# Leqr/MSMP-PDE

Measured on AMD Instinct MI355X. Metric: rollout-steps/sec (whole node), E2 nx=100 tw=25, higher is better.
Workload: dtype f32; 1 GPU; E2 MSMP-PDE (MP_PDE_SolverLEMLinGated), 2048 graphs x nx=100, time_window=25, 6 gated layer pairs, radius graph n=3; graphs_total=2048, graphs_per_gpu=2048, nodes_per_gpu=204800, edges_per_gpu=1204224, parallelism=dp1 (graph-sharded, no collective in the rollout), sub_batches=1, range_policy_switched_to_exact_fp32=False, preheat=163 untimed steps (>= 1 s) after the 5 warm-up steps

## Files before the change

### msmp-pde_amd/csrc/aux_kernels.hip

```cpp
#include <limits.h>
#include <stdarg.h>
#include <string.h>
#include "graph_norm.h"
#include <vector>
#include "mfma_tiles.h"

namespace msmp {

static thread_local char g_err[512] = "";

void set_error(const char* fmt, ...) {
    va_list ap;
    va_start(ap, fmt);
    vsnprintf(g_err, sizeof(g_err), fmt, ap);
    va_end(ap);
}

int check_launch(const char* what) {
    const hipError_t e = hipGetLastError();
    if (e != hipSuccess) {
        set_error("%s: %s", what, hipGetErrorString(e));
        return MSMP_ERR_HIP;
    }
    return MSMP_OK;
// ... 354 lines not shown
            (void)hipGetLastError();
            if (hipMalloc(&dp, sizeof(int)) == hipSuccess && hipMemset(dp, 0, sizeof(int)) == hipSuccess) {
                g_status_dev = static_cast<int*>(dp);
                g_status_mode = 2;
            } else {
                (void)hipGetLastError();
                g_status_mode = -1;
            }
        }
    }
    return g_status_dev;
}
}

extern "C" int msmp_last_status(int* flags_out, int reset) {
    MSMP_REQUIRE(flags_out, MSMP_ERR_ARG, "msmp_last_status: null pointer");
    int* dp = status_ptr();
    *flags_out = 0;
    if (g_status_mode == 1) {
        *flags_out = __atomic_load_n(g_status_host, __ATOMIC_RELAXED);
        if (reset) __atomic_store_n(g_status_host, 0, __ATOMIC_RELAXED);
    } else if (g_status_mode == 2) {
        hipError_t e = hipMemcpy(flags_out, dp, sizeof(int), hipMemcpyDeviceToHost);
        if (e == hipSuccess && reset) e = hipMemset(dp, 0, sizeof(int));
        MSMP_REQUIRE(e == hipSuccess, MSMP_ERR_HIP, "msmp_last_status: %s", hipGetErrorString(e));
    } else {
        MSMP_REQUIRE(false, MSMP_ERR_HIP, "msmp_last_status: no status word (allocation failed)");
    }
    return MSMP_OK;
}

extern "C" int msmp_version(void) { return MSMP_ABI_VERSION; }
extern "C" const char* msmp_last_error(void) { return g_err; }

struct TuneRow {
    const char* key;
    int value;
    int def;
    int lo, hi;
    bool flag;
    constexpr TuneRow(const char* k, int d, int l, int h, bool f) : key(k), value(d), def(d), lo(l), hi(h), flag(f) {}
};
#define ANY_INT INT_MIN, INT_MAX, false
#define ON_OFF INT_MIN, INT_MAX, true
static TuneRow g_tune[] = {
    {"split", 1, ANY_INT},
    {"edge_nb", 0, ANY_INT},
    {"pair", 1, ANY_INT},
    {"tile", 2, ANY_INT},
    {"tile_arith", 1, ANY_INT},
    {"tile_align", 0, ANY_INT},
    {"bwd_gemm", 1, ANY_INT},
    {"tail", 1, ANY_INT},
    {"lem_share", 1, 1, 16, false},
    {"lem_tail", 1, ON_OFF},
    {"lem_wide", 1, ON_OFF},
    {"wide_msg", 1, ON_OFF},
    {"wide_tail", 0, ON_OFF},
    {"wide_proj", 0, ON_OFF},
};
#undef ANY_INT
#undef ON_OFF

static TuneRow* tune_row(const char* key) {
    if (key)
        for (TuneRow& r : g_tune)
            if (!strcmp(key, r.key)) return &r;
    return nullptr;
}

int msmp_tune_get(const char* key) {
    const TuneRow* r = tune_row(key);
    return r ? r->value : 0;
}

extern "C" int msmp_tune_query(const char* key) { return msmp_tune_get(key); }

extern "C" int msmp_tune(const char* key, int value) {
    TuneRow* r = tune_row(key);
    MSMP_REQUIRE(r, MSMP_ERR_ARG, "msmp_tune: unknown key");
    MSMP_REQUIRE(value >= r->lo && value <= r->hi, MSMP_ERR_ARG, "msmp_tune: %s = %d is out of range (%d to %d)", key, value, r->lo, r->hi);
    r->value = r->flag ? value != 0 : value;
    return MSMP_OK;
}

extern "C" int64_t msmp_packed_layer_floats(int tw, int nv) {
    if (tw <= 0 || nv < 1 || nv > MSMP_MAX_VARS) return -1;
    return packed_layout(tw, nv).total;
}

extern "C" int msmp_pack_layer_f32(const float* w1, const float* b1, const float* w2, const float* b2,
                                   const float* w3, const float* b3, const float* w4, const float* b4,
                                   int tw, int nv, float* packed_out, msmp_stream_t stream) {
    MSMP_REQUIRE(w1 && b1 && w2 && b2 && w3 && b3 && w4 && b4 && packed_out, MSMP_ERR_ARG, "msmp_pack_layer_f32: null pointer");
    MSMP_REQUIRE(tw > 0 && nv >= 1 && nv <= MSMP_MAX_VARS, MSMP_ERR_ARG, "msmp_pack_layer_f32: bad tw=%d nv=%d", tw, nv);
    PackArgs a{w1, b1, w2, b2, w3, b3, w4, b4, tw, nv, packed_out};
    hipLaunchKernelGGL(pack_layer_kernel, dim3(256), dim3(256), 0, (hipStream_t)stream, a);
    hipLaunchKernelGGL(pack_layer_scale_kernel, dim3(4), dim3(256), 0, (hipStream_t)stream, a);
    hipLaunchKernelGGL(pack_layer_split_kernel, dim3(256), dim3(256), 0, (hipStream_t)stream, a);
    return check_launch("pack_layer_kernel");
}

extern "C" int msmp_scatter_mean_f32(const float* msg, const int32_t* rowptr, int64_t n_nodes, float* agg_out,
                                     msmp_stream_t stream) {
    MSMP_REQUIRE(rowptr && agg_out, MSMP_ERR_ARG, "msmp_scatter_mean_f32: null pointer");
    MSMP_REQUIRE(n_nodes > 0 && n_nodes < (1L << 31), MSMP_ERR_ARG, "msmp_scatter_mean_f32: bad n_nodes");
// ... 130 lines not shown
```

### msmp-pde_amd/csrc/mlp_kernels.hip

```cpp
#include "mfma_tiles.h"

namespace msmp {

struct EdgeArgs {
    const float* h;
    const float* u;
    const float* pos;
    const float* vars;
    const int* tgt;
    const int* col;
    const int* rowptr;
    long n_edges, n_nodes;
    int tile_nodes;
    int xcd_map;
    int tw, nv, nc1;
    const float* w1;
    const float* w2;
    const float* w2s;
    const float* scales;
    const float* b1;
    const float* b2;
    const float* P;
    const float* Q;
    float* msg;
// ... 783 lines not shown
        }
    }
#pragma unroll
    for (int T = 0; T < 4; ++T)
#pragma unroll
        for (int r = 0; r < 16; ++r) y[T][0][r] *= inv4;
}

__global__ __launch_bounds__(256, 2) void node_update_split_kernel(NodeSplitArgs sa) {
    __shared__ __attribute__((aligned(16))) float lds[2 * SPLIT_CHUNK_FLOATS];
    const NodeArgs& a = sa.b;
    const int tid = threadIdx.x, lane = tid & 63, wave = tid >> 6;
    const int c = lane & 31, hh = lane >> 5;
    const long n = (long)blockIdx.x * 128 + wave * 32 + c;
    const long nc = n < a.n_nodes ? n : a.n_nodes - 1;
    f32x16 y[4][1];
    node_head_split(a.h, a.agg, a.vars, nc, a.nv, a.b3, a.b4, a.w3v, sa.w3s, sa.scales, lds, tid, lane, hh, y);
    if (n < a.n_nodes) {
        float* o = a.out + (size_t)n * H + 4 * hh;
        const float* hx = a.h + (size_t)n * H + 4 * hh;
#pragma unroll
        for (int T = 0; T < 4; ++T)
#pragma unroll
            for (int q = 0; q < 4; ++q) {
                f32x4 v;
                if (a.mode == MSMP_LAYER_LIN) {
#pragma unroll
                    for (int m = 0; m < 4; ++m) v[m] = y[T][0][4 * q + m];
                } else {
                    const f32x4 x = *reinterpret_cast<const f32x4*>(hx + 32 * T + 8 * q);
#pragma unroll
                    for (int m = 0; m < 4; ++m) v[m] = x[m] + swishf(y[T][0][4 * q + m]);
                }
                *reinterpret_cast<f32x4*>(o + 32 * T + 8 * q) = v;
            }
    }
}

struct TailArgs {
    const float* h;
    const float* agg[2];
    const float* vars;
    const int* graph_ptr;
    int nv, mode;
    float eps;
    const float* b3[2];
    const float* b4[2];
    const float* w3vh[2];
    const float* w3s[2];
    const float* w4t[2];
    const float* scales[2];
    float* out;
    int* status;
};

constexpr float TAIL_ACT_SCALE = 64.0f;
constexpr float TAIL_NODE_SCALE = 256.0f;
__device__ __forceinline__ float tail_node_scaled(float x) { return __builtin_amdgcn_fmed3f(x * TAIL_NODE_SCALE, -65504.0f, 65504.0f); }

constexpr int ROWBUF_FLOATS = 128 * 32;
__device__ __forceinline__ void tail_rows_issue(const float* __restrict__ h, const float* __restrict__ agg, int n0, int n1, int ch, float* buf, int tid) {
    const float* src = (ch < 4 ? h : agg) + 32 * (ch & 3);
#pragma unroll
    for (int i = 0; i < 4; ++i) {
        const int P = tid + 256 * i, r = P >> 3;
        const int node = min(n0 + r, n1 - 1);
        const float* g = src + (size_t)node * H + 4 * ((P & 7) ^ ((r >> 1) & 7));
        __builtin_amdgcn_global_load_lds((const __attribute__((address_space(1))) void*)g, (__attribute__((address_space(3))) void*)(buf + 4 * P), 16, 0, 0);
    }
}
__device__ __forceinline__ void tail_rows_read(const float* buf, int row, int hh, f32x4 (&dst)[4]) {
    const float* rb = buf + row * 32;
    const int sw = (row >> 1) & 7;
#pragma unroll
    for (int s = 0; s < 2; ++s) {
        dst[2 * s] = *reinterpret_cast<const f32x4*>(rb + 4 * ((4 * s + 2 * hh) ^ sw));
        dst[2 * s + 1] = *reinterpret_cast<const f32x4*>(rb + 4 * ((4 * s + 2 * hh + 1) ^ sw));
    }
}

__device__ __forceinline__ void wstage_dma(const float* __restrict__ chunk, float* buf, int tid) {
#pragma unroll
    for (int i = 0; i < 4; ++i)
        __builtin_amdgcn_global_load_lds((const __attribute__((address_space(1))) void*)(chunk + 4 * (tid + 256 * i)),
                                         (__attribute__((address_space(3))) void*)(buf + 4 * (tid + 256 * i)), 16, 0, 0);
}

__device__ __forceinline__ void tail_bias_load(const float* b3, int hh, f32x16 (&z)[4][1]) {
#pragma unroll
    for (int T = 0; T < 4; ++T)
#pragma unroll
        for (int q = 0; q < 4; ++q) {
            const f32x4 bv = *reinterpret_cast<const f32x4*>(b3 + 32 * T + 8 * q + 4 * hh);
#pragma unroll
            for (int m = 0; m < 4; ++m) z[T][0][4 * q + m] = bv[m];
        }
}
__device__ __forceinline__ void tail_bias_pin(f32x16 (&z)[4][1]) {
#pragma unroll
    for (int T = 0; T < 4; ++T) asm volatile("" : "+v"(z[T][0]));
}
__device__ __forceinline__ void tail_bias_scale(f32x16 (&z)[4][1], float sc3) {
#pragma unroll
    for (int T = 0; T < 4; ++T)
#pragma unroll
        for (int r = 0; r < 16; ++r) z[T][0][r] *= sc3;
}
__device__ __forceinline__ float tail_sc3(const float* scales) { return uniform_ro(scales, 2) * TAIL_NODE_SCALE; }

__device__ __forceinline__ void tail_chunk_frags(const float* buf, int myrow, int hh, half8 (&bhi)[1][2], half8 (&blo)[1][2]) {
    f32x4 pf[4];
    tail_rows_read(buf, myrow, hh, pf);
#pragma unroll
    for (int s = 0; s < 2; ++s) {
        const f32x4 v0 = pf[2 * s], v1 = pf[2 * s + 1];
        const float v[8] = {v0[0], v0[1], v0[2], v0[3], v1[0], v1[1], v1[2], v1[3]};
        split8_node(v, bhi[0][s], blo[0][s]);
    }
}

template <int CH0, int PB>
__device__ __forceinline__ void head_chunks(float* rowbuf, int n0, int n1, const float* __restrict__ h, const float* __restrict__ agg, const float* w3vh,
                                            const float* w3s, const float* w4t, float* lds, int tid, int lane, int myrow, int hh, f32x16 (&z)[4][1],
                                            half8 (&wvf)[2][4] PROF_ARGS) {
#pragma unroll
    for (int ch = CH0; ch < 8; ++ch) {
        if (ch < 7) tail_rows_issue(h, agg, n0, n1, ch + 1, rowbuf + ((ch + 1) & 1) * ROWBUF_FLOATS, tid);
        wstage_dma(ch < 7 ? w3s + (size_t)(ch + 1) * SPLIT_CHUNK_FLOATS : w4t, lds + ((ch + 1) & 1) * SPLIT_CHUNK_FLOATS, tid);
        half8 bhi[1][2], blo[1][2];
        tail_chunk_frags(rowbuf + (ch & 1) * ROWBUF_FLOATS, myrow, hh, bhi, blo);
        if (ch == 5) {
            const half8* wv = reinterpret_cast<const half8*>(w3vh) + lane;
#pragma unroll
            for (int m = 0; m < 2; ++m)
#pragma unroll
                for (int T = 0; T < 4; ++T) wvf[m][T] = wv[(m * 4 + T) * 64];
        }
        PROF_MARK(PB);
        mma_chunk_split<1>(lds + (ch & 1) * SPLIT_CHUNK_FLOATS, lane, bhi, blo, z);
        PROF_MARK(PB + 1);
        __syncthreads();
        PROF_MARK(PB + 2);
    }
}

__device__ __forceinline__ void tail_var_frags(const float* xvl, int myrow, int hh, half8 (&bx)[2]) {
    const f32x4 x0 = *reinterpret_cast<const f32x4*>(xvl + 8 * myrow), x1 = *reinterpret_cast<const f32x4*>(xvl + 8 * myrow + 4);
    const float xr[8] = {x0[0], x0[1], x0[2], x0[3], x1[0], x1[1], x1[2], x1[3]};
    float xv[8];
#pragma unroll
    for (int f = 0; f < 8; ++f) xv[f] = tail_node_scaled(xr[f]);
    var_slot_frags(xv, hh, bx);
}

template <typename MidHook, typename LastHook>
__device__ __forceinline__ void head_finish(const float* b4, const float* w4t, const float* scales, float* lds, int tid, int lane, int c, int hh,
                                            f32x16 (&z)[4][1], const half8 (&wvf)[2][4], const half8 (&bx)[2], f32x16 (&yT)[4], MidHook mid_hook,
                                            LastHook last_hook, bool center, float* zref) {
    const float inv3 = uniform_ro(scales, 6) * (TAIL_ACT_SCALE / TAIL_NODE_SCALE), sc4 = uniform_ro(scales, 3) * TAIL_ACT_SCALE;
#pragma unroll
    for (int m = 0; m < 2; ++m)
#pragma unroll
        for (int T = 0; T < 4; ++T) z[T][0] = __builtin_amdgcn_mfma_f32_32x32x16_f16(wvf[m][T], bx[m], z[T][0], 0, 0, 0);
    mid_hook();
    __builtin_amdgcn_sched_barrier(0);
#pragma unroll
    for (int T = 0; T < 4; ++T)
#pragma unroll
        for (int r = 0; r < 16; ++r) {
#if MSMP_PRECISE_ACT
            z[T][0][r] = TAIL_ACT_SCALE * swishf(z[T][0][r] * inv3 * (1.0f / TAIL_ACT_SCALE));
#else
            const float xs = z[T][0][r] * inv3;
            const float e = __builtin_amdgcn_exp2f(xs * (-1.44269504088896340736f / TAIL_ACT_SCALE));
            z[T][0][r] = xs * __builtin_amdgcn_rcpf(1.0f + e);
#endif
        }

    if (center) {
        if ((tid >> 6) == 0 && c == 0) {
#pragma unroll
            for (int T = 0; T < 4; ++T)
#pragma unroll
                for (int q = 0; q < 4; ++q)
                    *reinterpret_cast<f32x4*>(zref + 32 * T + 8 * q + 4 * hh) = f32x4{z[T][0][4 * q], z[T][0][4 * q + 1], z[T][0][4 * q + 2], z[T][0][4 * q + 3]};
        }
        __syncthreads();
#pragma unroll
        for (int T = 0; T < 4; ++T)
#pragma unroll
            for (int q = 0; q < 4; ++q) {
                const f32x4 rv = *reinterpret_cast<const f32x4*>(zref + 32 * T + 8 * q + 4 * hh);
#pragma unroll
                for (int m = 0; m < 4; ++m) z[T][0][4 * q + m] -= rv[m];
            }
    }
    {
        const f32x4 bv = center ? f32x4{0.f, 0.f, 0.f, 0.f} : *reinterpret_cast<const f32x4*>(b4 + 4 * c) * sc4;
#pragma unroll
        for (int T = 0; T < 4; ++T)
#pragma unroll
            for (int r = 0; r < 16; ++r) yT[T][r] = bv[T];
    }
#pragma unroll
    for (int t = 0; t < 4; ++t) {
        if (t < 3) wstage_dma(w4t + (size_t)(t + 1) * SPLIT_CHUNK_FLOATS, lds + ((t + 1) & 1) * SPLIT_CHUNK_FLOATS, tid);
        else last_hook();
        __builtin_amdgcn_sched_barrier(0);
        half8 zhi[1][2], zlo[1][2];
        split_acc_tile<1>(z[t], zhi, zlo);
        const half8* w = reinterpret_cast<const half8*>(lds + (t & 1) * SPLIT_CHUNK_FLOATS) + lane;
#pragma unroll
        for (int s = 0; s < 2; ++s)
#pragma unroll
            for (int T = 0; T < 4; ++T) {
                const half8 whi = w[((s * 4 + T) * 2 + 0) * 64], wlo = w[((s * 4 + T) * 2 + 1) * 64];
                MSMP_MFMA_LOLO(1, yT[T], zlo[0][s], wlo);
                yT[T] = __builtin_amdgcn_mfma_f32_32x32x16_f16(zhi[0][s], wlo, yT[T], 0, 0, 0);
                yT[T] = __builtin_amdgcn_mfma_f32_32x32x16_f16(zlo[0][s], whi, yT[T], 0, 0, 0);
                yT[T] = __builtin_amdgcn_mfma_f32_32x32x16_f16(zhi[0][s], whi, yT[T], 0, 0, 0);
            }
        if (t < 3) __syncthreads();
    }
}

__device__ __forceinline__ void tile_t_total(const float (&v)[4], float* part, float* tot, int tid, int wave, int c, int hh,
                                             float (&out)[4]) {
#pragma unroll
    for (int T = 0; T < 4; ++T) part[(wave * 2 + hh) * H + 32 * T + c] = v[T];
    __syncthreads();
    if (tid < H) {
        float s = 0.f;
#pragma unroll
        for (int p = 0; p < 8; ++p) s += part[p * H + tid];
        tot[tid] = s;
    }
    __syncthreads();
#pragma unroll
    for (int T = 0; T < 4; ++T) out[T] = tot[32 * T + c];
}

__device__ __forceinline__ void tile_t_instance_norm(f32x16 (&x)[4], int wave, int cnt, float unit, float eps, float* part, float* tot,
                                                     int tid, int c, int hh, int* status) {
    const float inv = 1.0f / (float)max(cnt, 1);
    const bool ragged = wave * 32 + 32 > cnt;
    if (ragged) {
#pragma unroll
        for (int T = 0; T < 4; ++T)
#pragma unroll
            for (int r = 0; r < 16; ++r) x[T][r] = wave * 32 + acc_row(r, hh) < cnt ? x[T][r] : 0.f;
    }
    float s[4], m[4];
#pragma unroll
    for (int T = 0; T < 4; ++T) {
        float a0 = 0.f, a1 = 0.f;
#pragma unroll
        for (int r = 0; r < 16; r += 2) { a0 += x[T][r]; a1 += x[T][r + 1]; }
        s[T] = a0 + a1;
    }
    tile_t_total(s, part, tot, tid, wave, c, hh, m);
#pragma unroll
    for (int T = 0; T < 4; ++T) {
        const float mean = m[T] * inv;
        float a0 = 0.f, a1 = 0.f;
#pragma unroll
        for (int r = 0; r < 16; r += 2) {
            x[T][r] -= mean;
            x[T][r + 1] -= mean;
            if (ragged) {
                x[T][r] = wave * 32 + acc_row(r, hh) < cnt ? x[T][r] : 0.f;
                x[T][r + 1] = wave * 32 + acc_row(r + 1, hh) < cnt ? x[T][r + 1] : 0.f;
            }
            a0 = fmaf(x[T][r], x[T][r], a0);
            a1 = fmaf(x[T][r + 1], x[T][r + 1], a1);
        }
        s[T] = a0 + a1;
    }
    tile_t_total(s, part, tot, tid, wave, c, hh, m);
    if (wave == 0 && !(m[0] + m[1] + m[2] + m[3] < 3.0e38f)) status_raise(status, MSMP_STATUS_NONFINITE);
#pragma unroll
    for (int T = 0; T < 4; ++T) {
        const float f = unit * msmp_rsq(m[T] * inv * unit * unit + eps);
#pragma unroll
        for (int r = 0; r < 16; ++r) x[T][r] *= f;
    }
}

template <bool GATED>
__global__ __launch_bounds__(256, 2) void node_tail_split_kernel(TailArgs a) {
    __shared__ __attribute__((aligned(16))) float smem[2 * SPLIT_CHUNK_FLOATS + 2 * ROWBUF_FLOATS + 9 * H + 8 * 128];
    float* const lds = smem;
    float* const rowbuf = smem + 2 * SPLIT_CHUNK_FLOATS;
    float* const part = rowbuf + 2 * ROWBUF_FLOATS;
    float* const tot = part + 8 * H;
    float* const xvl = tot + H;
    const int tid = threadIdx.x, lane = tid & 63, wave = tid >> 6;
    const int c = lane & 31, hh = lane >> 5;
    const int n0 = a.graph_ptr[blockIdx.x], n1 = a.graph_ptr[blockIdx.x + 1];
    const int cnt = n1 - n0;
    if (cnt <= 0) return;

    PROF_DECL
#pragma unroll
    for (int i = 0; i < 4; ++i) {
        const int e = tid + 256 * i, row = e >> 3, f = e & 7;
        const float v = a.vars[(size_t)min(n0 + row, n1 - 1) * a.nv + min(f, a.nv - 1)];
        xvl[e] = v * (row < cnt && f < a.nv ? 1.0f : 0.f);
    }
    const int myrow = wave * 32 + c;
    f32x16 tau[4], y[4];
    f32x16 z[4][1];
    half8 wvf[2][4], bx[2];
    if (GATED) {
        f32x16 zg[4][1];
        tail_rows_issue(a.h, a.agg[1], n0, n1, 0, rowbuf, tid);
        wstage_dma(a.w3s[1], lds, tid);
        tail_bias_load(a.b3[1], hh, zg);
        tail_bias_load(a.b3[0], hh, z);
        tail_bias_pin(zg);
        tail_bias_pin(z);
        tail_bias_scale(zg, tail_sc3(a.scales[1]));
        tail_bias_scale(z, tail_sc3(a.scales[0]));
        __syncthreads();
        PROF_MARK(5);
        half8 bhi[1][2], blo[1][2];
#pragma unroll
        for (int s = 0; s < 8; ++s) {
            const int ch = s >> 1;
            if (!(s & 1)) {
                tail_rows_issue(a.h, a.agg[1], n0, n1, ch + 1, rowbuf + ((ch + 1) & 1) * ROWBUF_FLOATS, tid);
                wstage_dma(a.w3s[0] + (size_t)ch * SPLIT_CHUNK_FLOATS, lds + SPLIT_CHUNK_FLOATS, tid);
                __builtin_amdgcn_sched_barrier(0);
                tail_chunk_frags(rowbuf + (ch & 1) * ROWBUF_FLOATS, myrow, hh, bhi, blo);
                PROF_MARK(6);
                mma_chunk_split<1>(lds, lane, bhi, blo, zg);
            } else {
                wstage_dma(a.w3s[1] + (size_t)(ch + 1) * SPLIT_CHUNK_FLOATS, lds, tid);
                __builtin_amdgcn_sched_barrier(0);
                PROF_MARK(6);
                mma_chunk_split<1>(lds + SPLIT_CHUNK_FLOATS, lane, bhi, blo, z);
            }
            PROF_MARK(7);
            __syncthreads();
            PROF_MARK(8);
        }
        head_chunks<4, 9>(rowbuf, n0, n1, a.h, a.agg[1], a.w3vh[1], a.w3s[1], a.w4t[1], lds, tid, lane, myrow, hh, zg, wvf PROF_PASS);
        tail_var_frags(xvl, myrow, hh, bx);
        head_finish(a.b4[1], a.w4t[1], a.scales[1], lds, tid, lane, c, hh, zg, wvf, bx, tau,
                    [&] { tail_rows_issue(a.h, a.agg[0], n0, n1, 4, rowbuf, tid); },
                    [&] { wstage_dma(a.w3s[0] + (size_t)4 * SPLIT_CHUNK_FLOATS, lds, tid); }, true, tot);
        PROF_MARK(0);
        tile_t_instance_norm(tau, wave, cnt, uniform_ro(a.scales[1], 7) * (1.0f / TAIL_ACT_SCALE), a.eps, part, tot, tid, c, hh, a.status);
#pragma unroll
        for (int T = 0; T < 4; ++T)
#pragma unroll
            for (int r = 0; r < 16; ++r) tau[T][r] = sigmoidf_(tau[T][r]);
        __syncthreads();
        PROF_MARK(1);
        head_chunks<4, 12>(rowbuf, n0, n1, a.h, a.agg[0], a.w3vh[0], a.w3s[0], a.w4t[0], lds, tid, lane, myrow, hh, z, wvf PROF_PASS);
    } else {
        tail_rows_issue(a.h, a.agg[0], n0, n1, 0, rowbuf, tid);
        wstage_dma(a.w3s[0], lds, tid);
        tail_bias_load(a.b3[0], hh, z);
        tail_bias_pin(z);
        tail_bias_scale(z, tail_sc3(a.scales[0]));
        __syncthreads();
        PROF_MARK(5);
        head_chunks<0, 12>(rowbuf, n0, n1, a.h, a.agg[0], a.w3vh[0], a.w3s[0], a.w4t[0], lds, tid, lane, myrow, hh, z, wvf PROF_PASS);
        tail_var_frags(xvl, myrow, hh, bx);
    }
    head_finish(a.b4[0], a.w4t[0], a.scales[0], lds, tid, lane, c, hh, z, wvf, bx, y, [] {}, [] {}, GATED || a.mode == MSMP_LAYER_LIN, tot);
    PROF_MARK(2);
    const size_t base = ((size_t)n0 + wave * 32 + 4 * hh) * H + 4 * c;
    const int lim = cnt - wave * 32 - 4 * hh;
    const bool full = wave * 32 + 32 <= cnt;
    const bool need_h = GATED || a.mode != MSMP_LAYER_LIN;
    f32x4 hx[16];
    if (need_h) {
        if (full) {
#pragma unroll
            for (int r = 0; r < 16; ++r) hx[r] = *reinterpret_cast<const f32x4*>(a.h + base + (size_t)((r & 3) + 8 * (r >> 2)) * H);
        } else {
#pragma unroll
            for (int r = 0; r < 16; ++r) {
                const int row = (r & 3) + 8 * (r >> 2);
                hx[r] = row < lim ? *reinterpret_cast<const f32x4*>(a.h + base + (size_t)row * H) : f32x4{0.f, 0.f, 0.f, 0.f};
            }
        }
    }
    float unit = uniform_ro(a.scales[0], 7) * (1.0f / TAIL_ACT_SCALE);
    if (!GATED && a.mode != MSMP_LAYER_LIN) {
#pragma unroll
        for (int T = 0; T < 4; ++T)
#pragma unroll
            for (int r = 0; r < 16; ++r) y[T][r] = hx[r][T] + swishf(y[T][r] * unit);
        unit = 1.0f;
    }
    tile_t_instance_norm(y, wave, cnt, unit, a.eps, part, tot, tid, c, hh, a.status);
    if (need_h) {
        float mx = 0.f;
#pragma unroll
        for (int r = 0; r < 16; ++r) mx = fmaxf(fmaxf(fmaxf(fabsf(hx[r][0]), fabsf(hx[r][1])), fmaxf(fabsf(hx[r][2]), fabsf(hx[r][3]))), mx);
        if (mx > NODE_RANGE) status_raise(a.status, MSMP_STATUS_NODE_SATURATED);
    }
    PROF_MARK(3);
    if (GATED) {
#pragma unroll
        for (int T = 0; T < 4; ++T)
#pragma unroll
            for (int r = 0; r < 16; ++r) y[T][r] = fmaf(tau[T][r], swishf(y[T][r]) - hx[r][T], hx[r][T]);
    }
    if (full) {
#pragma unroll
        for (int r = 0; r < 16; ++r)
            *reinterpret_cast<f32x4*>(a.out + base + (size_t)((r & 3) + 8 * (r >> 2)) * H) = f32x4{y[0][r], y[1][r], y[2][r], y[3][r]};
    } else {
#pragma unroll
        for (int r = 0; r < 16; ++r) {
            const int row = (r & 3) + 8 * (r >> 2);
            if (row < lim) *reinterpret_cast<f32x4*>(a.out + base + (size_t)row * H) = f32x4{y[0][r], y[1][r], y[2][r], y[3][r]};
        }
    }
    PROF_MARK(4);
    PROF_FLUSH
}

}

using namespace msmp;


extern "C" int msmp_edge_mlp_f32(const float* h, const float* u, const float* pos, const float* vars,
                                 const int32_t* tgt, const int32_t* col, int64_t n_nodes, int64_t n_edges,
                                 int tw, int nv, const float* packed, float* msg_out, msmp_stream_t stream) {
    MSMP_REQUIRE(h && u && pos && vars && tgt && col && packed && msg_out, MSMP_ERR_ARG, "msmp_edge_mlp_f32: null pointer");
    MSMP_REQUIRE(n_nodes > 0 && n_edges >= 0 && tw > 0 && nv >= 1 && nv <= MSMP_MAX_VARS, MSMP_ERR_ARG,
                 "msmp_edge_mlp_f32: bad sizes N=%ld E=%ld tw=%d nv=%d", (long)n_nodes, (long)n_edges, tw, nv);
    MSMP_REQUIRE(n_edges < (1L << 31) && n_nodes < (1L << 31), MSMP_ERR_UNSUPPORTED, "msmp_edge_mlp_f32: int32 index range");
    if (n_edges == 0) return MSMP_OK;
    const PackedLayout L = packed_layout(tw, nv);
    EdgeArgs a{h, u, pos, vars, tgt, col, nullptr, (long)n_edges, (long)n_nodes, 0, 0, tw, nv, L.nc1,
               packed + L.w1, packed + L.w2, packed + L.w2s, packed + L.scales, packed + L.b1, packed + L.b2, nullptr, nullptr, msg_out, nullptr, msmp_tune_get("split") ? status_ptr() : nullptr};
    constexpr int NB = 2;
    const unsigned grid = (unsigned)((n_edges + 128 * NB - 1) / (128 * NB));
    timing_begin(MSMP_K_EDGE_MLP, (hipStream_t)stream);
    hipLaunchKernelGGL((edge_mlp_kernel<NB, false, false>), dim3(grid), dim3(256), 0, (hipStream_t)stream, a);
    timing_end(MSMP_K_EDGE_MLP, (hipStream_t)stream);
    return check_launch("edge_mlp_kernel");
}

extern "C" int msmp_node_project_f32(const float* h, const float* u, const float* pos, const float* vars, int64_t n_nodes,
                                     int tw, int nv, const float* packed, float* p_out, float* q_out, msmp_stream_t stream) {
    MSMP_REQUIRE(h && u && pos && vars && packed && p_out && q_out, MSMP_ERR_ARG, "msmp_node_project_f32: null pointer");
    MSMP_REQUIRE(n_nodes > 0 && n_nodes < (1L << 31) && tw > 0 && nv >= 1 && nv <= MSMP_MAX_VARS, MSMP_ERR_ARG,
                 "msmp_node_project_f32: bad sizes");
    const PackedLayout L = packed_layout(tw, nv);
    ProjArgs a{h, u, pos, vars, (long)n_nodes, tw, nv, L.nc1, packed + L.w1, packed + L.b1, p_out, q_out};
    const unsigned grid = (unsigned)((n_nodes + 127) / 128);
    timing_begin(MSMP_K_NODE_PROJ, (hipStream_t)stream);
    if (msmp_tune_get("split")) {
        ProjSplitArgs sa{a, packed + L.w1t, packed + L.scales};
        hipLaunchKernelGGL(node_proj_split_kernel, dim3(grid), dim3(256), 0, (hipStream_t)stream, sa);
    } else
        hipLaunchKernelGGL(node_proj_kernel, dim3(grid), dim3(256), 0, (hipStream_t)stream, a);
    timing_end(MSMP_K_NODE_PROJ, (hipStream_t)stream);
    return check_launch("node_proj_kernel");
}

constexpr int64_t PAIR_MAX_NODES = 65536;

static int edge_aggregate(const float* h, const float* u, const float* pos, const float* vars, const float* P, const float* Q,
                          const int32_t* rowptr, const int32_t* col, const int32_t* tgt, int64_t n_nodes, int64_t n_edges,
                          int max_in_degree, int tw, int nv, const float* packed, float* agg_out, msmp_stream_t stream,
                          const char* who) {
    MSMP_REQUIRE(rowptr && col && tgt && packed && agg_out, MSMP_ERR_ARG, "%s: null pointer", who);
    MSMP_REQUIRE(n_nodes > 0 && n_edges >= 0 && tw > 0 && nv >= 1 && nv <= MSMP_MAX_VARS && max_in_degree >= 0, MSMP_ERR_ARG,
                 "%s: bad sizes", who);
// ... 30 lines not shown
    if (!pair || (pair == 1 && n_nodes > PAIR_MAX_NODES)) return MSMP_ERR_UNSUPPORTED;
    if (!msmp_tune_get("split") || msmp_tune_get("edge_nb") == 2) return MSMP_ERR_UNSUPPORTED;
    if (n_edges <= 0 || max_in_degree <= 0 || max_in_degree > 128 || n_edges >= (1L << 31) || n_nodes >= (1L << 31)) return MSMP_ERR_UNSUPPORTED;
    const PackedLayout L = packed_layout(tw, nv);
    hipStream_t st = (hipStream_t)stream;
    ProjSplitArgs2 pa;
    const float* packed[2] = {packed_a, packed_b};
    float* pp[2] = {p_a, p_b};
    float* qq[2] = {q_a, q_b};
    float* agg[2] = {agg_a, agg_b};
    for (int i = 0; i < 2; ++i)
        pa.head[i] = ProjSplitArgs{ProjArgs{h, u, pos, vars, (long)n_nodes, tw, nv, L.nc1, packed[i] + L.w1, packed[i] + L.b1, pp[i], qq[i]},
                                   packed[i] + L.w1t, packed[i] + L.scales};
    timing_begin(MSMP_K_NODE_PROJ, st);
    hipLaunchKernelGGL(node_proj_split_pair_kernel, dim3((unsigned)((n_nodes + 127) / 128), 2), dim3(256), 0, st, pa);
    timing_end(MSMP_K_NODE_PROJ, st);
    int tile_nodes = 128 / max_in_degree;
    if (tile_nodes > 256) tile_nodes = 256;
    EdgeArgs2 ea;
    for (int i = 0; i < 2; ++i)
        ea.head[i] = EdgeArgs{nullptr, nullptr, nullptr, nullptr, tgt, col, rowptr, (long)n_edges, (long)n_nodes, tile_nodes, 0, tw, nv, L.nc1,
                              packed[i] + L.w1, packed[i] + L.w2, packed[i] + L.w2s, packed[i] + L.scales, packed[i] + L.b1,
                              packed[i] + L.b2, pp[i], qq[i], nullptr, agg[i], status_ptr()};
    timing_begin(MSMP_K_EDGE_MLP, st);
    hipLaunchKernelGGL(edge_mlp_pair_kernel_occ2, dim3((unsigned)((n_nodes + tile_nodes - 1) / tile_nodes), 2), dim3(256), 0, st, ea);
    timing_end(MSMP_K_EDGE_MLP, st);
    return check_launch("edge_mlp_pair_kernel_occ2");
}

extern "C" int msmp_edge_aggregate_f32(const float* h, const float* u, const float* pos, const float* vars,
                                       const int32_t* rowptr, const int32_t* col, const int32_t* tgt, int64_t n_nodes,
                                       int64_t n_edges, int max_in_degree, int tw, int nv, const float* packed,
                                       float* agg_out, msmp_stream_t stream) {
    MSMP_REQUIRE(h && u && pos && vars, MSMP_ERR_ARG, "msmp_edge_aggregate_f32: null pointer");
    return edge_aggregate(h, u, pos, vars, nullptr, nullptr, rowptr, col, tgt, n_nodes, n_edges, max_in_degree, tw, nv, packed,
                          agg_out, stream, "msmp_edge_aggregate_f32");
}

extern "C" int msmp_edge_aggregate_projected_f32(const float* p, const float* q, const int32_t* rowptr, const int32_t* col,
                                                 const int32_t* tgt, int64_t n_nodes, int64_t n_edges, int max_in_degree,
                                                 int tw, int nv, const float* packed, float* agg_out, msmp_stream_t stream) {
    MSMP_REQUIRE(p && q, MSMP_ERR_ARG, "msmp_edge_aggregate_projected_f32: null pointer");
    return edge_aggregate(nullptr, nullptr, nullptr, nullptr, p, q, rowptr, col, tgt, n_nodes, n_edges, max_in_degree, tw, nv,
                          packed, agg_out, stream, "msmp_edge_aggregate_projected_f32");
}

#if MSMP_PROF
extern "C" __attribute__((visibility("default"))) int msmp_debug_prof(unsigned long long* out16, int reset) {
    if (reset) { unsigned long long z[16] = {0}; return (int)hipMemcpyToSymbol(HIP_SYMBOL(g_prof), z, sizeof(z)); }
    return (int)hipMemcpyFromSymbol(out16, HIP_SYMBOL(g_prof), 16 * sizeof(unsigned long long));
}
#endif

extern "C" int msmp_node_tail_f32(const float* h, const float* agg_main, const float* agg_gate, const float* vars,
                                  const int32_t* graph_ptr, int64_t n_nodes, int64_t n_graphs, int max_graph_nodes, int nv,
                                  const float* packed_main, const float* packed_gate, int mode, float eps, float* out,
                                  msmp_stream_t stream) {
    MSMP_REQUIRE(h && agg_main && vars && graph_ptr && packed_main && out, MSMP_ERR_ARG, "msmp_node_tail_f32: null pointer");
    MSMP_REQUIRE((agg_gate != nullptr) == (packed_gate != nullptr), MSMP_ERR_ARG, "msmp_node_tail_f32: give both gate arguments or none");
    MSMP_REQUIRE(n_nodes > 0 && n_graphs > 0 && n_graphs < (1L << 31) && nv >= 1 && nv <= MSMP_MAX_VARS, MSMP_ERR_ARG,
                 "msmp_node_tail_f32: bad sizes");
    MSMP_REQUIRE(mode == MSMP_LAYER_LIN || mode == MSMP_LAYER_RESIDUAL_SWISH, MSMP_ERR_ARG, "msmp_node_tail_f32: bad mode %d", mode);
    MSMP_REQUIRE(!packed_gate || mode == MSMP_LAYER_LIN, MSMP_ERR_ARG, "msmp_node_tail_f32: the gated pair uses GNN_LayerLin layers");
    MSMP_REQUIRE(out != h, MSMP_ERR_ARG, "msmp_node_tail_f32: out may not alias h");
    MSMP_REQUIRE(max_graph_nodes > 0 && max_graph_nodes <= 128, MSMP_ERR_UNSUPPORTED,
                 "msmp_node_tail_f32: graphs of up to 128 nodes (got max_graph_nodes=%d); use the piecewise entry points", max_graph_nodes);
    MSMP_REQUIRE(msmp_tune_get("split"), MSMP_ERR_UNSUPPORTED, "msmp_node_tail_f32: only on the fp16-split matrix path");
    const PackedLayout L = packed_layout(1, nv);
    const float* pg = packed_gate ? packed_gate : packed_main;
    TailArgs a{h, {agg_main, agg_gate}, vars, graph_ptr, nv, mode, eps,
               {packed_main + L.b3, pg + L.b3}, {packed_main + L.b4, pg + L.b4}, {packed_main + L.w3vh, pg + L.w3vh},
               {packed_main + L.w3s, pg + L.w3s}, {packed_main + L.w4t, pg + L.w4t}, {packed_main + L.scales, pg + L.scales}, out, status_ptr()};
    timing_begin(MSMP_K_NODE_UPDATE, (hipStream_t)stream);
    if (packed_gate) hipLaunchKernelGGL(node_tail_split_kernel<true>, dim3((unsigned)n_graphs), dim3(256), 0, (hipStream_t)stream, a);
    else hipLaunchKernelGGL(node_tail_split_kernel<false>, dim3((unsigned)n_graphs), dim3(256), 0, (hipStream_t)stream, a);
    timing_end(MSMP_K_NODE_UPDATE, (hipStream_t)stream);
    return check_launch("node_tail_split_kernel");
}

extern "C" int msmp_node_update_f32(const float* h, const float* agg, const float* vars, int64_t n_nodes, int nv,
                                    const float* packed, int mode, float* out, msmp_stream_t stream) {
    MSMP_REQUIRE(h && agg && vars && packed && out, MSMP_ERR_ARG, "msmp_node_update_f32: null pointer");
    MSMP_REQUIRE(n_nodes > 0 && nv >= 1 && nv <= MSMP_MAX_VARS, MSMP_ERR_ARG, "msmp_node_update_f32: bad sizes");
    MSMP_REQUIRE(mode == MSMP_LAYER_LIN || mode == MSMP_LAYER_RESIDUAL_SWISH, MSMP_ERR_ARG, "msmp_node_update_f32: bad mode %d", mode);
    MSMP_REQUIRE(out != h, MSMP_ERR_ARG, "msmp_node_update_f32: out may not alias h");
    const PackedLayout L = packed_layout(1, nv);
    NodeArgs a{h, agg, vars, (long)n_nodes, nv, mode, packed + L.w3, packed + L.w4,
               packed + L.b3, packed + L.b4, packed + L.w3v, out};
    constexpr int NB = 1;
    const unsigned grid = (unsigned)((n_nodes + 128 * NB - 1) / (128 * NB));
    timing_begin(MSMP_K_NODE_UPDATE, (hipStream_t)stream);
    if (msmp_tune_get("split")) {
        NodeSplitArgs sa{a, packed + L.w3s, packed + L.scales};
        hipLaunchKernelGGL(node_update_split_kernel, dim3(grid), dim3(256), 0, (hipStream_t)stream, sa);
    } else
        hipLaunchKernelGGL(node_update_kernel<NB>, dim3(grid), dim3(256), 0, (hipStream_t)stream, a);
    timing_end(MSMP_K_NODE_UPDATE, (hipStream_t)stream);
    return check_launch("node_update_kernel");
}
```

Baseline: 161.4 rollout-steps/s.

## Make node tail kernel persistent with next-graph prologue prefetch

```diff
diff --git a/msmp-pde_amd/csrc/aux_kernels.hip b/msmp-pde_amd/csrc/aux_kernels.hip
--- a/msmp-pde_amd/csrc/aux_kernels.hip
+++ b/msmp-pde_amd/csrc/aux_kernels.hip
@@ -430,6 +430,7 @@
     {"tile_align", 0, ANY_INT},
     {"bwd_gemm", 1, ANY_INT},
     {"tail", 1, ANY_INT},
+    {"tail_grid", 0, 0, INT_MAX, false},
     {"lem_share", 1, 1, 16, false},
     {"lem_tail", 1, ON_OFF},
     {"lem_wide", 1, ON_OFF},
diff --git a/msmp-pde_amd/csrc/mlp_kernels.hip b/msmp-pde_amd/csrc/mlp_kernels.hip
--- a/msmp-pde_amd/csrc/mlp_kernels.hip
+++ b/msmp-pde_amd/csrc/mlp_kernels.hip
@@ -859,6 +859,7 @@
     const float* scales[2];
     float* out;
     int* status;
+    unsigned n_graphs;
 };
 
 constexpr float TAIL_ACT_SCALE = 64.0f;
@@ -867,12 +868,12 @@
 
 constexpr int ROWBUF_FLOATS = 128 * 32;
 __device__ __forceinline__ void tail_rows_issue(const float* __restrict__ h, const float* __restrict__ agg, int n0, int n1, int ch, float* buf, int tid) {
-    const float* src = (ch < 4 ? h : agg) + 32 * (ch & 3);
+    const float* src = (ch < 4 ? h : agg) + (size_t)n0 * H + 32 * (ch & 3);
 #pragma unroll
     for (int i = 0; i < 4; ++i) {
         const int P = tid + 256 * i, r = P >> 3;
-        const int node = min(n0 + r, n1 - 1);
-        const float* g = src + (size_t)node * H + 4 * ((P & 7) ^ ((r >> 1) & 7));
+        const unsigned row = (unsigned)min(r, n1 - n0 - 1);
+        const float* g = src + (row * (unsigned)H + 4u * (unsigned)((P & 7) ^ ((r >> 1) & 7)));
         __builtin_amdgcn_global_load_lds((const __attribute__((address_space(1))) void*)g, (__attribute__((address_space(3))) void*)(buf + 4 * P), 16, 0, 0);
     }
 }
@@ -893,26 +894,6 @@
                                          (__attribute__((address_space(3))) void*)(buf + 4 * (tid + 256 * i)), 16, 0, 0);
 }
 
-__device__ __forceinline__ void tail_bias_load(const float* b3, int hh, f32x16 (&z)[4][1]) {
-#pragma unroll
-    for (int T = 0; T < 4; ++T)
-#pragma unroll
-        for (int q = 0; q < 4; ++q) {
-            const f32x4 bv = *reinterpret_cast<const f32x4*>(b3 + 32 * T + 8 * q + 4 * hh);
-#pragma unroll
-            for (int m = 0; m < 4; ++m) z[T][0][4 * q + m] = bv[m];
-        }
-}
-__device__ __forceinline__ void tail_bias_pin(f32x16 (&z)[4][1]) {
-#pragma unroll
-    for (int T = 0; T < 4; ++T) asm volatile("" : "+v"(z[T][0]));
-}
-__device__ __forceinline__ void tail_bias_scale(f32x16 (&z)[4][1], float sc3) {
-#pragma unroll
-    for (int T = 0; T < 4; ++T)
-#pragma unroll
-        for (int r = 0; r < 16; ++r) z[T][0][r] *= sc3;
-}
 __device__ __forceinline__ float tail_sc3(const float* scales) { return uniform_ro(scales, 2) * TAIL_NODE_SCALE; }
 
 __device__ __forceinline__ void tail_chunk_frags(const float* buf, int myrow, int hh, half8 (&bhi)[1][2], half8 (&blo)[1][2]) {
@@ -934,6 +915,7 @@
     for (int ch = CH0; ch < 8; ++ch) {
         if (ch < 7) tail_rows_issue(h, agg, n0, n1, ch + 1, rowbuf + ((ch + 1) & 1) * ROWBUF_FLOATS, tid);
         wstage_dma(ch < 7 ? w3s + (size_t)(ch + 1) * SPLIT_CHUNK_FLOATS : w4t, lds + ((ch + 1) & 1) * SPLIT_CHUNK_FLOATS, tid);
+        __builtin_amdgcn_sched_barrier(0);
         half8 bhi[1][2], blo[1][2];
         tail_chunk_frags(rowbuf + (ch & 1) * ROWBUF_FLOATS, myrow, hh, bhi, blo);
         if (ch == 5) {
@@ -951,12 +933,12 @@
     }
 }
 
-__device__ __forceinline__ void tail_var_frags(const float* xvl, int myrow, int hh, half8 (&bx)[2]) {
+__device__ __forceinline__ void tail_var_frags(const float* xvl, int myrow, int hh, int cnt, int nv, half8 (&bx)[2]) {
     const f32x4 x0 = *reinterpret_cast<const f32x4*>(xvl + 8 * myrow), x1 = *reinterpret_cast<const f32x4*>(xvl + 8 * myrow + 4);
     const float xr[8] = {x0[0], x0[1], x0[2], x0[3], x1[0], x1[1], x1[2], x1[3]};
     float xv[8];
 #pragma unroll
-    for (int f = 0; f < 8; ++f) xv[f] = tail_node_scaled(xr[f]);
+    for (int f = 0; f < 8; ++f) xv[f] = tail_node_scaled(xr[f] * (myrow < cnt && f < nv ? 1.0f : 0.f));
     var_slot_frags(xv, hh, bx);
 }
 
@@ -1031,18 +1013,19 @@
     }
 }
 
+__device__ __forceinline__ void tail_lds_barrier() { asm volatile("s_waitcnt lgkmcnt(0)\n\ts_barrier" ::: "memory"); }
 __device__ __forceinline__ void tile_t_total(const float (&v)[4], float* part, float* tot, int tid, int wave, int c, int hh,
                                              float (&out)[4]) {
 #pragma unroll
     for (int T = 0; T < 4; ++T) part[(wave * 2 + hh) * H + 32 * T + c] = v[T];
-    __syncthreads();
+    tail_lds_barrier();
     if (tid < H) {
         float s = 0.f;
 #pragma unroll
         for (int p = 0; p < 8; ++p) s += part[p * H + tid];
         tot[tid] = s;
     }
-    __syncthreads();
+    tail_lds_barrier();
 #pragma unroll
     for (int T = 0; T < 4; ++T) out[T] = tot[32 * T + c];
 }
@@ -1092,6 +1075,137 @@
         for (int r = 0; r < 16; ++r) x[T][r] *= f;
     }
 }
+
+__device__ __forceinline__ bool tail_graph_at(const TailArgs& a, unsigned& g, unsigned stride, int& n0, int& n1) {
+    const __attribute__((address_space(4))) int* gp = (const __attribute__((address_space(4))) int*)a.graph_ptr;
+    for (; g < a.n_graphs; g += stride) {
+        n0 = gp[g];
+        n1 = gp[g + 1];
+        if (n1 > n0) return true;
+    }
+    return false;
+}
+
+__device__ __forceinline__ void tail_vars_issue(const TailArgs& a, int n0, int n1, float* xvl, int tid) {
+#pragma unroll
+    for (int i = 0; i < 4; ++i) {
+        const int e = tid + 256 * i, row = e >> 3, f = e & 7;
+        const float* g = a.vars + (size_t)n0 * a.nv + (unsigned)(min(row, n1 - n0 - 1) * a.nv + min(f, a.nv - 1));
+        __builtin_amdgcn_global_load_lds((const __attribute__((address_space(1))) void*)g, (__attribute__((address_space(3))) void*)(xvl + e), 4, 0, 0);
+    }
+}
+
+template <bool GATED>
+__device__ __forceinline__ void tail_prologue_request(const TailArgs& a, int n0, int n1, float* lds, float* rowbuf, float* xvl, int tid) {
+    tail_rows_issue(a.h, a.agg[GATED ? 1 : 0], n0, n1, 0, rowbuf, tid);
+    wstage_dma(a.w3s[GATED ? 1 : 0], lds, tid);
+    tail_vars_issue(a, n0, n1, xvl, tid);
+    __builtin_amdgcn_sched_barrier(0);
+}
+template <bool GATED>
+__device__ __forceinline__ float tail_bias_element(const TailArgs& a, int tid) {
+    const int k = GATED ? 1 - (tid >> 7) : 0;
+    return a.b3[k][tid & 127] * tail_sc3(a.scales[k]);
+}
+__device__ __forceinline__ void tail_bias_read(const float* staged, int hh, f32x16 (&z)[4][1]) {
+#pragma unroll
+    for (int T = 0; T < 4; ++T)
+#pragma unroll
+        for (int q = 0; q < 4; ++q) {
+            const f32x4 bv = *reinterpret_cast<const f32x4*>(staged + 32 * T + 8 * q + 4 * hh);
+#pragma unroll
+            for (int m = 0; m < 4; ++m) z[T][0][4 * q + m] = bv[m];
+        }
+}
+
+__device__ __forceinline__ void tail_requests_landed() { asm volatile("s_waitcnt vmcnt(0)" ::: "memory"); }
+
+__device__ __forceinline__ int tail_tid_again(int wave_s) {
+    int l;
+    asm volatile("v_mbcnt_lo_u32_b32 %0, -1, 0\n\tv_mbcnt_hi_u32_b32 %0, -1, %0" : "=v"(l));
+    return wave_s * 64 + (l & 63);
+}
+
+__device__ __forceinline__ float tail_swish_minus(float y, float h, bool fused) {
+#if MSMP_PRECISE_ACT
+    return swishf(y) - h;
+#else
+    const float rc = __builtin_amdgcn_rcpf(1.0f + __builtin_amdgcn_exp2f(y * -1.44269504088896340736f));
+    if (fused) return __builtin_fmaf(y, rc, -h);
+    {
+#pragma clang fp contract(off)
+        const float t = y * rc;
+        return t - h;
+    }
+#endif
+}
+
+template <bool GATED>
+__device__ __forceinline__ void tail_end(const TailArgs& a, int n0, int n1, bool more, f32x16 (&y)[4], f32x16 (&tau)[4], float* part, float* tot,
+                                         int wave_s PROF_ARGS) {
+    const int tid = tail_tid_again(wave_s), lane = tid & 63, wave = tid >> 6, c = lane & 31, hh = lane >> 5;
+    const int cnt = n1 - n0;
+    const float* const hg = a.h + (size_t)n0 * H;
+    float* const og = a.out + (size_t)n0 * H;
+    const unsigned base = (unsigned)((wave * 32 + 4 * hh) * H + 4 * c);
+    const int lim = cnt - wave * 32 - 4 * hh;
+    const bool full = wave * 32 + 32 <= cnt;
+    const bool need_h = GATED || a.mode != MSMP_LAYER_LIN;
+    const float bias_el = more ? tail_bias_element<GATED>(a, tid) : 0.f;
+    f32x4 hx[16];
+    if (need_h) {
+        if (full) {
+#pragma unroll
+            for (int r = 0; r < 16; ++r) hx[r] = *reinterpret_cast<const f32x4*>(hg + (base + (unsigned)(((r & 3) + 8 * (r >> 2)) * H)));
+        } else {
+#pragma unroll
+            for (int r = 0; r < 16; ++r) {
+                const int row = (r & 3) + 8 * (r >> 2);
+                hx[r] = row < lim ? *reinterpret_cast<const f32x4*>(hg + (base + (unsigned)(row * H))) : f32x4{0.f, 0.f, 0.f, 0.f};
+            }
+        }
+    }
+    float unit = uniform_ro(a.scales[0], 7) * (1.0f / TAIL_ACT_SCALE);
+    if (!GATED && a.mode != MSMP_LAYER_LIN) {
+#pragma unroll
+        for (int T = 0; T < 4; ++T)
+#pragma unroll
+            for (int r = 0; r < 16; ++r) y[T][r] = hx[r][T] + swishf(y[T][r] * unit);
+        unit = 1.0f;
+    }
+    tile_t_instance_norm(y, wave, cnt, unit, a.eps, part, tot, tid, c, hh, a.status);
+    if (need_h) {
+        float mx = 0.f;
+#pragma unroll
+        for (int r = 0; r < 16; ++r) mx = fmaxf(fmaxf(fmaxf(fabsf(hx[r][0]), fabsf(hx[r][1])), fmaxf(fabsf(hx[r][2]), fabsf(hx[r][3]))), mx);
+        if (mx > NODE_RANGE) status_raise(a.status, MSMP_STATUS_NODE_SATURATED);
+    }
+    PROF_MARK(3);
+    if (GATED) {
+#pragma unroll
+        for (int T = 0; T < 4; ++T) {
+#pragma unroll
+            for (int r = 0; r < 16; ++r) y[T][r] = fmaf(tau[T][r], tail_swish_minus(y[T][r], hx[r][T], r != 15), hx[r][T]);
+            asm volatile("" : "+v"(y[T]));
+        }
+    }
+    if (more) {
+        part[tid] = bias_el;
+        tail_requests_landed();
+    }
+    if (full) {
+#pragma unroll
+        for (int r = 0; r < 16; ++r)
+            *reinterpret_cast<f32x4*>(og + (base + (unsigned)(((r & 3) + 8 * (r >> 2)) * H))) = f32x4{y[0][r], y[1][r], y[2][r], y[3][r]};
+    } else {
+#pragma unroll
+        for (int r = 0; r < 16; ++r) {
+            const int row = (r & 3) + 8 * (r >> 2);
+            if (row < lim) *reinterpret_cast<f32x4*>(og + (base + (unsigned)(row * H))) = f32x4{y[0][r], y[1][r], y[2][r], y[3][r]};
+        }
+    }
+}
+
 
 template <bool GATED>
 __global__ __launch_bounds__(256, 2) void node_tail_split_kernel(TailArgs a) {
@@ -1101,135 +1215,108 @@
     float* const part = rowbuf + 2 * ROWBUF_FLOATS;
     float* const tot = part + 8 * H;
     float* const xvl = tot + H;
-    const int tid = threadIdx.x, lane = tid & 63, wave = tid >> 6;
-    const int c = lane & 31, hh = lane >> 5;
-    const int n0 = a.graph_ptr[blockIdx.x], n1 = a.graph_ptr[blockIdx.x + 1];
-    const int cnt = n1 - n0;
-    if (cnt <= 0) return;
+    unsigned g = blockIdx.x;
+    int n0, n1;
+    if (!tail_graph_at(a, g, gridDim.x, n0, n1)) return;
 
     PROF_DECL
-#pragma unroll
-    for (int i = 0; i < 4; ++i) {
-        const int e = tid + 256 * i, row = e >> 3, f = e & 7;
-        const float v = a.vars[(size_t)min(n0 + row, n1 - 1) * a.nv + min(f, a.nv - 1)];
-        xvl[e] = v * (row < cnt && f < a.nv ? 1.0f : 0.f);
-    }
-    const int myrow = wave * 32 + c;
-    f32x16 tau[4], y[4];
-    f32x16 z[4][1];
-    half8 wvf[2][4], bx[2];
-    if (GATED) {
-        f32x16 zg[4][1];
-        tail_rows_issue(a.h, a.agg[1], n0, n1, 0, rowbuf, tid);
-        wstage_dma(a.w3s[1], lds, tid);
-        tail_bias_load(a.b3[1], hh, zg);
-        tail_bias_load(a.b3[0], hh, z);
-        tail_bias_pin(zg);
-        tail_bias_pin(z);
-        tail_bias_scale(zg, tail_sc3(a.scales[1]));
-        tail_bias_scale(z, tail_sc3(a.scales[0]));
-        __syncthreads();
-        PROF_MARK(5);
-        half8 bhi[1][2], blo[1][2];
-#pragma unroll
-        for (int s = 0; s < 8; ++s) {
-            const int ch = s >> 1;
-            if (!(s & 1)) {
-                tail_rows_issue(a.h, a.agg[1], n0, n1, ch + 1, rowbuf + ((ch + 1) & 1) * ROWBUF_FLOATS, tid);
-                wstage_dma(a.w3s[0] + (size_t)ch * SPLIT_CHUNK_FLOATS, lds + SPLIT_CHUNK_FLOATS, tid);
-                __builtin_amdgcn_sched_barrier(0);
-                tail_chunk_frags(rowbuf + (ch & 1) * ROWBUF_FLOATS, myrow, hh, bhi, blo);
-                PROF_MARK(6);
-                mma_chunk_split<1>(lds, lane, bhi, blo, zg);
-            } else {
-                wstage_dma(a.w3s[1] + (size_t)(ch + 1) * SPLIT_CHUNK_FLOATS, lds, tid);
-                __builtin_amdgcn_sched_barrier(0);
-                PROF_MARK(6);
-                mma_chunk_split<1>(lds + SPLIT_CHUNK_FLOATS, lane, bhi, blo, z);
-            }
-            PROF_MARK(7);
+#if MSMP_PROF
+    unsigned long long prof_graphs = 0;
+#endif
+    const int wave_s = __builtin_amdgcn_readfirstlane(threadIdx.x >> 6) & 3;
+    {
+        const int tid = threadIdx.x;
+        tail_prologue_request<GATED>(a, n0, n1, lds, rowbuf, xvl, tid);
+        part[tid] = tail_bias_element<GATED>(a, tid);
+        tail_requests_landed();
+    }
+    for (;;) {
+        int zero_v = 0;
+        asm volatile("" : "+v"(zero_v));
+        const int zero = __builtin_amdgcn_readfirstlane(zero_v);
+        const float* const w3s[2] = {a.w3s[0] + zero, a.w3s[1] + zero};
+        const float* const w4t[2] = {a.w4t[0] + zero, a.w4t[1] + zero};
+        const int tid = tail_tid_again(wave_s);
+        const int lane = tid & 63, wave = tid >> 6;
+        const int c = lane & 31, hh = lane >> 5;
+        const int cnt = n1 - n0;
+        const int myrow = wave * 32 + c;
+        unsigned gn = g + gridDim.x;
+        int nn0 = 0, nn1 = 0;
+        const bool more = tail_graph_at(a, gn, gridDim.x, nn0, nn1);
+        auto next_prologue = [&] { if (more) tail_prologue_request<GATED>(a, nn0, nn1, lds, rowbuf, xvl, tail_tid_again(wave_s)); };
+        f32x16 tau[4], y[4];
+        f32x16 z[4][1];
+        half8 wvf[2][4], bx[2];
+        tail_lds_barrier();
+        if (GATED) {
+            f32x16 zg[4][1];
+            tail_bias_read(part, hh, zg);
+            tail_bias_read(part + H, hh, z);
+            PROF_MARK(5);
+            half8 bhi[1][2], blo[1][2];
+#pragma unroll
+            for (int s = 0; s < 8; ++s) {
+                const int ch = s >> 1;
+                if (!(s & 1)) {
+                    tail_rows_issue(a.h, a.agg[1], n0, n1, ch + 1, rowbuf + ((ch + 1) & 1) * ROWBUF_FLOATS, tid);
+                    wstage_dma(w3s[0] + (size_t)ch * SPLIT_CHUNK_FLOATS, lds + SPLIT_CHUNK_FLOATS, tid);
+                    __builtin_amdgcn_sched_barrier(0);
+                    tail_chunk_frags(rowbuf + (ch & 1) * ROWBUF_FLOATS, myrow, hh, bhi, blo);
+                    PROF_MARK(6);
+                    mma_chunk_split<1>(lds, lane, bhi, blo, zg);
+                } else {
+                    wstage_dma(w3s[1] + (size_t)(ch + 1) * SPLIT_CHUNK_FLOATS, lds, tid);
+                    __builtin_amdgcn_sched_barrier(0);
+                    PROF_MARK(6);
+                    mma_chunk_split<1>(lds + SPLIT_CHUNK_FLOATS, lane, bhi, blo, z);
+                }
+                PROF_MARK(7);
+                __syncthreads();
+                PROF_MARK(8);
+            }
+            head_chunks<4, 9>(rowbuf, n0, n1, a.h, a.agg[1], a.w3vh[1], w3s[1], w4t[1], lds, tid, lane, myrow, hh, zg, wvf PROF_PASS);
+            tail_var_frags(xvl, myrow, hh, cnt, a.nv, bx);
+            head_finish(a.b4[1], w4t[1], a.scales[1], lds, tid, lane, c, hh, zg, wvf, bx, tau,
+                        [&] { tail_rows_issue(a.h, a.agg[0], n0, n1, 4, rowbuf, tid); },
+                        [&] { wstage_dma(w3s[0] + (size_t)4 * SPLIT_CHUNK_FLOATS, lds, tid); }, true, tot);
+            PROF_MARK(0);
+            tile_t_instance_norm(tau, wave, cnt, uniform_ro(a.scales[1], 7) * (1.0f / TAIL_ACT_SCALE), a.eps, part, tot, tid, c, hh, a.status);
+#pragma unroll
+            for (int T = 0; T < 4; ++T)
+#pragma unroll
+                for (int r = 0; r < 16; ++r) tau[T][r] = sigmoidf_(tau[T][r]);
             __syncthreads();
-            PROF_MARK(8);
-        }
-        head_chunks<4, 9>(rowbuf, n0, n1, a.h, a.agg[1], a.w3vh[1], a.w3s[1], a.w4t[1], lds, tid, lane, myrow, hh, zg, wvf PROF_PASS);
-        tail_var_frags(xvl, myrow, hh, bx);
-        head_finish(a.b4[1], a.w4t[1], a.scales[1], lds, tid, lane, c, hh, zg, wvf, bx, tau,
-                    [&] { tail_rows_issue(a.h, a.agg[0], n0, n1, 4, rowbuf, tid); },
-                    [&] { wstage_dma(a.w3s[0] + (size_t)4 * SPLIT_CHUNK_FLOATS, lds, tid); }, true, tot);
-        PROF_MARK(0);
-        tile_t_instance_norm(tau, wave, cnt, uniform_ro(a.scales[1], 7) * (1.0f / TAIL_ACT_SCALE), a.eps, part, tot, tid, c, hh, a.status);
-#pragma unroll
-        for (int T = 0; T < 4; ++T)
-#pragma unroll
-            for (int r = 0; r < 16; ++r) tau[T][r] = sigmoidf_(tau[T][r]);
-        __syncthreads();
-        PROF_MARK(1);
-        head_chunks<4, 12>(rowbuf, n0, n1, a.h, a.agg[0], a.w3vh[0], a.w3s[0], a.w4t[0], lds, tid, lane, myrow, hh, z, wvf PROF_PASS);
-    } else {
-        tail_rows_issue(a.h, a.agg[0], n0, n1, 0, rowbuf, tid);
-        wstage_dma(a.w3s[0], lds, tid);
-        tail_bias_load(a.b3[0], hh, z);
-        tail_bias_pin(z);
-        tail_bias_scale(z, tail_sc3(a.scales[0]));
-        __syncthreads();
-        PROF_MARK(5);
-        head_chunks<0, 12>(rowbuf, n0, n1, a.h, a.agg[0], a.w3vh[0], a.w3s[0], a.w4t[0], lds, tid, lane, myrow, hh, z, wvf PROF_PASS);
-        tail_var_frags(xvl, myrow, hh, bx);
-    }
-    head_finish(a.b4[0], a.w4t[0], a.scales[0], lds, tid, lane, c, hh, z, wvf, bx, y, [] {}, [] {}, GATED || a.mode == MSMP_LAYER_LIN, tot);
-    PROF_MARK(2);
-    const size_t base = ((size_t)n0 + wave * 32 + 4 * hh) * H + 4 * c;
-    const int lim = cnt - wave * 32 - 4 * hh;
-    const bool full = wave * 32 + 32 <= cnt;
-    const bool need_h = GATED || a.mode != MSMP_LAYER_LIN;
-    f32x4 hx[16];
-    if (need_h) {
-        if (full) {
-#pragma unroll
-            for (int r = 0; r < 16; ++r) hx[r] = *reinterpret_cast<const f32x4*>(a.h + base + (size_t)((r & 3) + 8 * (r >> 2)) * H);
+            PROF_MARK(1);
+            {
+                const int tid = tail_tid_again(wave_s), lane = tid & 63, hh = lane >> 5, myrow = (tid >> 6) * 32 + (lane & 31);
+                head_chunks<4, 12>(rowbuf, n0, n1, a.h, a.agg[0], a.w3vh[0], w3s[0], w4t[0], lds, tid, lane, myrow, hh, z, wvf PROF_PASS);
+                tail_var_frags(xvl, myrow, hh, cnt, a.nv, bx);
+            }
         } else {
-#pragma unroll
-            for (int r = 0; r < 16; ++r) {
-                const int row = (r & 3) + 8 * (r >> 2);
-                hx[r] = row < lim ? *reinterpret_cast<const f32x4*>(a.h + base + (size_t)row * H) : f32x4{0.f, 0.f, 0.f, 0.f};
-            }
-        }
-    }
-    float unit = uniform_ro(a.scales[0], 7) * (1.0f / TAIL_ACT_SCALE);
-    if (!GATED && a.mode != MSMP_LAYER_LIN) {
-#pragma unroll
-        for (int T = 0; T < 4; ++T)
-#pragma unroll
-            for (int r = 0; r < 16; ++r) y[T][r] = hx[r][T] + swishf(y[T][r] * unit);
-        unit = 1.0f;
-    }
-    tile_t_instance_norm(y, wave, cnt, unit, a.eps, part, tot, tid, c, hh, a.status);
-    if (need_h) {
-        float mx = 0.f;
-#pragma unroll
-        for (int r = 0; r < 16; ++r) mx = fmaxf(fmaxf(fmaxf(fabsf(hx[r][0]), fabsf(hx[r][1])), fmaxf(fabsf(hx[r][2]), fabsf(hx[r][3]))), mx);
-        if (mx > NODE_RANGE) status_raise(a.status, MSMP_STATUS_NODE_SATURATED);
-    }
-    PROF_MARK(3);
-    if (GATED) {
-#pragma unroll
-        for (int T = 0; T < 4; ++T)
-#pragma unroll
-            for (int r = 0; r < 16; ++r) y[T][r] = fmaf(tau[T][r], swishf(y[T][r]) - hx[r][T], hx[r][T]);
-    }
-    if (full) {
-#pragma unroll
-        for (int r = 0; r < 16; ++r)
-            *reinterpret_cast<f32x4*>(a.out + base + (size_t)((r & 3) + 8 * (r >> 2)) * H) = f32x4{y[0][r], y[1][r], y[2][r], y[3][r]};
-    } else {
-#pragma unroll
-        for (int r = 0; r < 16; ++r) {
-            const int row = (r & 3) + 8 * (r >> 2);
-            if (row < lim) *reinterpret_cast<f32x4*>(a.out + base + (size_t)row * H) = f32x4{y[0][r], y[1][r], y[2][r], y[3][r]};
-        }
-    }
-    PROF_MARK(4);
-    PROF_FLUSH
+            tail_bias_read(part, hh, z);
+            PROF_MARK(5);
+            head_chunks<0, 12>(rowbuf, n0, n1, a.h, a.agg[0], a.w3vh[0], w3s[0], w4t[0], lds, tid, lane, myrow, hh, z, wvf PROF_PASS);
+            tail_var_frags(xvl, myrow, hh, cnt, a.nv, bx);
+        }
+        head_finish(a.b4[0], w4t[0], a.scales[0], lds, tid, lane, c, hh, z, wvf, bx, y, [] {}, next_prologue, GATED || a.mode == MSMP_LAYER_LIN, tot);
+        PROF_MARK(2);
+        tail_end<GATED>(a, n0, n1, more, y, tau, part, tot, wave_s PROF_PASS);
+        PROF_MARK(4);
+#if MSMP_PROF
+        ++prof_graphs;
+#endif
+        if (!more) break;
+        g = gn;
+        n0 = nn0;
+        n1 = nn1;
+    }
+#if MSMP_PROF
+    if (threadIdx.x == 0 && (blockIdx.x & 15) == 0) {
+        for (int i_ = 0; i_ < 15; ++i_) atomicAdd(&g_prof[i_], (unsigned long long)pacc[i_]);
+        atomicAdd(&g_prof[15], prof_graphs);
+    }
+#endif
 }
 
 }
@@ -1366,6 +1453,18 @@
 }
 #endif
 
+static unsigned tail_grid(int64_t n_graphs) {
+    const int v = msmp_tune_get("tail_grid");
+    int64_t wgs = n_graphs;
+    if (v == 1) {
+        int dev = 0, cus = 0;
+        if (hipGetDevice(&dev) != hipSuccess || hipDeviceGetAttribute(&cus, hipDeviceAttributeMultiprocessorCount, dev) != hipSuccess || cus <= 0) cus = 256;
+        wgs = 2 * (int64_t)cus;
+    } else if (v >= 2)
+        wgs = v;
+    return (unsigned)(wgs < n_graphs ? wgs : n_graphs);
+}
+
 extern "C" int msmp_node_tail_f32(const float* h, const float* agg_main, const float* agg_gate, const float* vars,
                                   const int32_t* graph_ptr, int64_t n_nodes, int64_t n_graphs, int max_graph_nodes, int nv,
                                   const float* packed_main, const float* packed_gate, int mode, float eps, float* out,
@@ -1384,10 +1483,11 @@
     const float* pg = packed_gate ? packed_gate : packed_main;
     TailArgs a{h, {agg_main, agg_gate}, vars, graph_ptr, nv, mode, eps,
                {packed_main + L.b3, pg + L.b3}, {packed_main + L.b4, pg + L.b4}, {packed_main + L.w3vh, pg + L.w3vh},
-               {packed_main + L.w3s, pg + L.w3s}, {packed_main + L.w4t, pg + L.w4t}, {packed_main + L.scales, pg + L.scales}, out, status_ptr()};
+               {packed_main + L.w3s, pg + L.w3s}, {packed_main + L.w4t, pg + L.w4t}, {packed_main + L.scales, pg + L.scales}, out, status_ptr(), (unsigned)n_graphs};
+    const unsigned grid = tail_grid(n_graphs);
     timing_begin(MSMP_K_NODE_UPDATE, (hipStream_t)stream);
-    if (packed_gate) hipLaunchKernelGGL(node_tail_split_kernel<true>, dim3((unsigned)n_graphs), dim3(256), 0, (hipStream_t)stream, a);
-    else hipLaunchKernelGGL(node_tail_split_kernel<false>, dim3((unsigned)n_graphs), dim3(256), 0, (hipStream_t)stream, a);
+    if (packed_gate) hipLaunchKernelGGL(node_tail_split_kernel<true>, dim3(grid), dim3(256), 0, (hipStream_t)stream, a);
+    else hipLaunchKernelGGL(node_tail_split_kernel<false>, dim3(grid), dim3(256), 0, (hipStream_t)stream, a);
     timing_end(MSMP_K_NODE_UPDATE, (hipStream_t)stream);
     return check_launch("node_tail_split_kernel");
 }
```

Result: no change. 161.9 rollout-steps/s, median of 4 (+0.3%).
